# johnmartinsson/differentiable-mel-spectrogram

Measured on AMD Instinct MI355X. Metric: spectrogram frames/sec (fwd+bwd), higher is better.
Workload: dtype f32

## Files before the change

differentiable-mel-spectrogram_amd/build.py:

```python
from __future__ import annotations

import glob
import os
import shutil
import subprocess
import sys

PKG_DIR = os.path.dirname(os.path.abspath(__file__))
CSRC = os.path.join(PKG_DIR, "csrc")
LIB_PATH = os.path.join(PKG_DIR, "libdmel_hip.so")
TORCH_LIB_PATH = os.path.join(PKG_DIR, "libdmel_torch.so")
OBJ_DIR = os.path.join(PKG_DIR, "build")
SPLIT_SOURCES = ["dmel_fwd.hip", "dmel_fwd_len.hip", "dmel_fwd_band.hip", "dmel_fwd_multi_len.hip", "dmel_fwd_band_len.hip", "dmel_fwd_fb_len.hip"]
FWD_PARTS = 4
SOURCES = SPLIT_SOURCES + ["dmel_aux.hip", "dmel_big.hip", "dmel_xgrad.hip", "dmel_xgrad_len.hip", "dmel_xgrad_band.hip", "dmel_xgrad_klen.hip", "dmel_pcen.hip", "dmel_bandnorm.hip", "dmel_specmask.hip", "dmel_deltas.hip", "dmel_statspool.hip", "dmel_attnpool.hip", "dmel_api.cpp", "dmel_tables.cpp", "dmel_comm.cpp"]
PUBLIC_HEADER = os.path.join(os.path.dirname(PKG_DIR), "include", "dmel.h")
HEADERS = sorted(glob.glob(os.path.join(CSRC, "*.h")) + glob.glob(os.path.join(CSRC, "*.inc"))) + [PUBLIC_HEADER]
FLAGS = ["--offload-arch=gfx950", "-O3", "-fPIC", "-std=c++17", "-Wall", "-Wno-unused-function"]


def _hipcc() -> str:
    for cand in (os.environ.get("HIPCC"), shutil.which("hipcc"), "/opt/rocm/bin/hipcc"):
        if cand and os.path.exists(cand):
            return cand
    raise RuntimeError("hipcc not found (set HIPCC or install ROCm)")


def _stale(target: str, deps) -> bool:
    if not os.path.exists(target):
        return True
    t = os.path.getmtime(target)
    return any(os.path.getmtime(d) > t for d in deps)


def _units():
    for src in SOURCES:
        sp = os.path.join(CSRC, src)
        stem = os.path.splitext(src)[0]
        if src in SPLIT_SOURCES:
            for k in range(FWD_PARTS):
                yield sp, os.path.join(OBJ_DIR, f"{stem}_part{k}.o"), ["-DDMEL_FWD_SPLIT", f"-DDMEL_FWD_PART={k}"]
        else:
            yield sp, os.path.join(OBJ_DIR, stem + ".o"), []


def _reap(procs) -> None:
    for pr in procs:
        if pr.poll() is None:
            pr.kill()
    for pr in procs:
        pr.wait()


def build(force: bool = False, verbose: bool = False) -> str:
    os.makedirs(OBJ_DIR, exist_ok=True)
    hipcc = _hipcc()
    objs, running = [], []
    jobs = max(1, min(int(os.environ.get("DMEL_BUILD_JOBS", "0")) or (os.cpu_count() or 2), 8))
    for sp, obj, extra in _units():
        objs.append(obj)
        if force or _stale(obj, [sp] + HEADERS):
            cmd = [hipcc] + FLAGS + extra + ["-x", "hip", "-c", sp, "-o", obj]
            if verbose:
                print(" ".join(cmd), flush=True)
            while len(running) >= jobs:
                if running.pop(0).wait() != 0:
                    _reap(running)
                    raise RuntimeError("hipcc failed")
            running.append(subprocess.Popen(cmd))
    while running:
        if running.pop(0).wait() != 0:
            _reap(running)
            raise RuntimeError("hipcc failed")
    if force or _stale(LIB_PATH, objs):
        cmd = [hipcc, "--offload-arch=gfx950", "-shared", "-fPIC", "-o", LIB_PATH] + objs + ["-ldl"]
        if verbose:
            print(" ".join(cmd), flush=True)
        subprocess.check_call(cmd)
    build_torch(force=force, verbose=verbose)
    return LIB_PATH


def build_torch(force: bool = False, verbose: bool = False) -> str:
    import importlib.util
    spec = importlib.util.find_spec("torch")
    if spec is None or not spec.submodule_search_locations:
        raise RuntimeError("torch is not importable: libdmel_torch.so cannot be built")
    tdir = list(spec.submodule_search_locations)[0]
    src = os.path.join(CSRC, "dmel_torch.cpp")
    if not (force or _stale(TORCH_LIB_PATH, [src, PUBLIC_HEADER, LIB_PATH])):
        return TORCH_LIB_PATH
    cxx = os.environ.get("CXX") or shutil.which("g++") or shutil.which("c++")
    if not cxx:
        raise RuntimeError("no C++ compiler found for libdmel_torch.so")
    inc = os.path.join(tdir, "include")
    cmd = [cxx, "-O2", "-fPIC", "-shared", "-std=c++17", "-D__HIP_PLATFORM_AMD__=1", "-DUSE_ROCM=1", "-D_GLIBCXX_USE_CXX11_ABI=1",
           "-I" + inc, "-I" + os.path.join(inc, "torch", "csrc", "api", "include"), "-I/opt/rocm/include",
           src, "-o", TORCH_LIB_PATH, "-L" + PKG_DIR, "-ldmel_hip", "-L" + os.path.join(tdir, "lib"),
# ... 10 lines not shown
```

differentiable-mel-spectrogram_amd/csrc/dmel_api.cpp:

```cpp
#include "../../include/dmel.h"
#include "dmel_kernels.h"
#include "dmel_lamtrack.h"
#include "dmel_stage.h"
#include "dmel_tables.h"

#include <algorithm>
#include <cmath>
#include <cstdio>
#include <cstdlib>
#include <cstring>
#include <functional>
#include <initializer_list>
#include <map>
#include <mutex>
#include <string>
#include <unordered_set>
#include <vector>

namespace {

thread_local std::string g_err;

dmel_status fail(dmel_status st, const std::string& msg)
{
// ... 432 lines not shown
    bp.split = split ? 1 : 0; bp.wodd = wodd;
    DMEL_HIP(dmel::launch_big(bp, s));
    prof_span(pl, m1, prof_mark(pl, s), 1);
    info->kernel_path = 3; info->frames_per_tile = pair ? 2 : 1; info->grid_fwd = grid;
    info->fb_blocks = 0; info->fb_blocks_dense = 0; info->lds_bytes = dmel::big_uses_global(bt.M) ? 0 : bt.M * 8;
    info->contraction = -1; info->wl_steps = 0;
    return DMEL_OK;
}

dmel_status forward_naive(dmel_plan* pl, NfftTables* tb, const dmel::LamArgs& lam, const FwdCall& c, const Scratch& sc, hipStream_t s,
                          dmel_plan_info* info)
{
    const int N = tb->n_fft;
    dmel::NaiveParams np{};
    np.x = c.x_direct(); np.x_ind = c.x_cell(); np.out = c.out; np.tangent = c.tangent; np.psum = sc.psum; np.win2 = sc.win; np.fb = tb->fb_dense;
    np.B = c.batch; np.L = pl->cfg.n_points; np.T = pl->T; np.hop = pl->cfg.hop_length; np.M = pl->cfg.n_mels;
    np.nchunks = pl->nchunks; np.N = N; np.F = tb->F; np.mode = c.mode;
    np.inv_L = 1.0f / (float)pl->cfg.n_points; np.eps = (float)c.eps; np.flags = c.flags; np.remove_dc = c.remove_dc; np.lam = lam;
    DMEL_HIP(dmel::launch_naive(np, s));
    info->kernel_path = 1; info->frames_per_tile = 1; info->grid_fwd = c.batch * pl->T;
    info->fb_blocks = 0; info->fb_blocks_dense = 0; info->lds_bytes = (2 * N + 2 * tb->F) * 4;
    info->contraction = -1; info->wl_steps = 0;
    return DMEL_OK;
}

dmel_status forward_fused(dmel_plan* pl, NfftTables* tb, const dmel::LamArgs& lam, const FwdCall& c, const Scratch& sc, hipStream_t s,
                          bool kernel_mean, dmel_plan_info* info)
{
    const int N = tb->n_fft;
    const MultiLaunch* ml = c.multi() ? &c.ml : nullptr;
    int mode = c.mode;
    const unsigned flags = c.flags & ~DMEL_FLAG_X_INDIRECT;
    dmel::FwdParams fp{};
    fp.x = c.x_direct(); fp.x_ind = c.x_cell(); fp.out = c.out; fp.tangent = c.tangent; fp.psum = (c.remove_dc && !kernel_mean) ? sc.psum : nullptr; fp.win2 = sc.win;
    fp.tw1 = dmel::mode_pairs(mode) ? tb->tw1p : tb->tw1; fp.tw2 = dmel::mode_pairs(mode) ? tb->tw2p : tb->tw2; fp.ent_b = tb->ent_b; fp.tile_ranges = tb->tile_ranges; fp.ent_b_floats = tb->ent_b_floats; fp.ent_pre = tb->ent_pre;
    for (int i = 0; i < 16; ++i) fp.pre_groups[i] = tb->pre_groups[i];
    fp.B = c.batch; fp.L = pl->cfg.n_points; fp.T = pl->T; fp.hop = pl->cfg.hop_length; fp.M = pl->cfg.n_mels;
    fp.nchunks = pl->nchunks; fp.groups = tb->groups; fp.xch_groups = tb->xch_groups;
    const bool hsplit = (flags & DMEL_FLAG_MFMA_BF16X3) && mode == dmel::kTrain && tb->ent_h != nullptr && (!c.lengths || c.fb_len);
    if (hsplit) mode = dmel::kTrainH;
    static const int wlc_env = std::getenv("DMEL_WLC") ? std::atoi(std::getenv("DMEL_WLC")) : -1;
    const bool wl_compact = tb->wl_total4 * 4 <= 320;
    if (mode == dmel::kTrain && tb->wl_b4 != nullptr && wlc_env != 0 && (wl_compact || wlc_env > 0)) {
        const int wide_fpt = dmel::forward_has_wlc_wide(N) ? dmel::forward_frames_per_tile(N, dmel::kTrainWW) : 0;
        const bool wide = wide_fpt > 0 && wlc_env == 2 && !c.lengths;
        mode = wide ? dmel::kTrainWW : dmel::kTrainW;
        fp.wl_b4 = tb->wl_b4; fp.wl_lane = tb->wl_lane; fp.wl_phases = tb->wl_phases; fp.wl_total4 = tb->wl_total4;
        for (int i = 0; i < dmel::kWlMaxPhases; ++i) { fp.wl_len4[i] = tb->wl_len4[i]; fp.wl_mg[i] = tb->wl_mg[i]; }
        fp.wl_merge = tb->wl_merge;
    }
    const int fpt = dmel::forward_frames_per_tile(N, mode);
    fp.tiles_per_clip = (pl->T + fpt - 1) / fpt;
    fp.inv_L = 1.0f / (float)pl->cfg.n_points; fp.eps = (float)c.eps; fp.flags = flags; fp.lam = lam;
    fp.remove_dc = c.remove_dc; fp.normalize = pl->cfg.normalize_window; fp.win_half = c.win_half;
    fp.spec_out = c.spec_out;
    fp.ent_h = tb->ent_h; fp.fb_nyq = tb->fb_nyq;
    static const int force_tpw = std::getenv("DMEL_TILES_PER_WG") ? std::atoi(std::getenv("DMEL_TILES_PER_WG")) : 0;
    int tpw = dmel::forward_tiles_per_wg(N, mode, c.batch, fp.tiles_per_clip);
    if (force_tpw == 1 || (force_tpw == 2 && dmel::forward_two_tiles(N, mode))) tpw = force_tpw;
    if (hsplit || c.lengths || (ml && ml->edges)) tpw = 1;
    fp.wgs_per_clip = (fp.tiles_per_clip + tpw - 1) / tpw;
    long long grid = (long long)c.batch * fp.wgs_per_clip;
    if (ml) {
        fp.ch_out = ml->ch_out; fp.ch_grid = (int)grid; fp.ch_list = ml->list; fp.ch_roles = ml->roles;
        for (int ch = 0; ch < dmel::kMaxChannels; ++ch) fp.ch_val[ch] = ml->vals[ch];
        grid *= ml->count;
    }
    if (grid > 0x7fffffffLL) return fail(DMEL_ERR_INVALID_ARGUMENT, "too many tiles for one launch");
    if (grid <= dmel::forward_resident_workgroups(N, mode)) fp.flags |= dmel::kFwdEdgeFirst;
    const bool band = ml && ml->edges;
    dmel::FwdLenParams lp{};
    lp.lengths = c.lengths;
    dmel::FwdMultiLenParams mlp{};
    mlp.lengths = c.lengths;
    dmel::FwdBandParams bp{};
    dmel::FwdBandLenParams blp{};
    blp.lengths = c.lengths;
    dmel::FwdFbLenParams flp{};
    flp.lengths = c.lengths;
    const bool fbk = c.fb_len && !ml && (mode == dmel::kTrain || mode == dmel::kTrainH || mode == dmel::kSpec);
    if (c.lengths && c.spec_out && !fbk) return fail(DMEL_ERR_UNSUPPORTED, "per-clip lengths: the spectrogram is saved by the kTrain / kTrainH kernels of a trained bank only");
    for (int ch = 0; band && ch <= dmel::kMaxChannels; ++ch) blp.band_edges[ch] = bp.band_edges[ch] = ml->edges[std::min(ch, ml->channels)];
    auto launch = [&](auto& q) { static_cast<dmel::FwdParams&>(q) = fp; return dmel::launch_forward(N, mode, tpw, q, (int)grid, s); };
    DMEL_HIP(c.lengths ? (band ? launch(blp) : ml ? launch(mlp) : fbk ? launch(flp) : launch(lp)) : band ? launch(bp) : launch(fp));
    info->kernel_path = 0; info->frames_per_tile = fpt; info->grid_fwd = (int)grid;
    info->fb_blocks = tb->n_entries; info->fb_blocks_dense = tb->n_dense;
    info->lds_bytes = dmel::forward_lds_bytes(N, mode);
    const bool spec_only = mode == dmel::kSpec || mode == dmel::kSpecTrain;
    info->contraction = spec_only ? -1 : (dmel::mode_wlc(mode) ? 1 : (mode == dmel::kTrainH ? 2 : 0));
    info->wl_steps = dmel::mode_wlc(mode) ? 4 * fp.wl_total4 : 0;
    return DMEL_OK;
}

dmel_status launch_forward_n(dmel_plan* pl, int N, const dmel::LamArgs& lam, const FwdCall& c, const Scratch& sc, hipStream_t s, bool* sums_done)
{
    if (N < 1) return fail(DMEL_ERR_UNSUPPORTED, "n_fft = " + std::to_string(N));
    const bool pow2 = (N & (N - 1)) == 0;
    const bool big = !pow2 || N > dmel::kMaxNfft;
    if (c.lengths && (big || N < dmel::kMinFastNfft || ((c.spec_out || c.mode == dmel::kSpec) && !c.fb_len) || c.win_half))
        return fail(DMEL_ERR_UNSUPPORTED, "per-clip lengths run the fused kernel only: n_fft 32 ... 16384 (n_fft = " + std::to_string(N) + ")");
    if (c.multi() && (big || N < dmel::kMinFastNfft || c.spec_out))
        return fail(DMEL_ERR_UNSUPPORTED, "the multi-window layer runs n_fft 32 ... 16384 only (n_fft = " + std::to_string(N) + ")");
    if (c.spec_out && (big || N < dmel::kMinFastNfft || c.mode != dmel::kTrain))
        return fail(DMEL_ERR_UNSUPPORTED, "the spectrogram is saved by the fused training kernel only (power-of-two n_fft from 32 to 16384, tangent requested)");
    if (big && (N & 1)) return fail(DMEL_ERR_UNSUPPORTED, "n_fft = " + std::to_string(N) + " is odd");
    NfftTables* tb = nullptr;
    dmel_status st = build_tables(pl, N, &tb);
    if (st != DMEL_OK) return st;
    dmel_plan_info info{};
    info.n_fft = N; info.n_freqs = tb->F; info.n_time = pl->T;
    if (big) {
        if ((st = forward_big(pl, tb, lam, c, sc, s, sums_done, &info)) == DMEL_OK) pl->info = info;
        return st;
    }
    const bool fast = N >= dmel::kMinFastNfft && N <= dmel::kMaxFastNfft;
    const bool kernel_mean = fast && pl->cfg.n_points <= 32768;
    const bool need_sums = c.remove_dc && !kernel_mean && !*sums_done;
    const bool need_window = !fast || !dmel::forward_window_in_lds(N);
    const size_t m0 = prof_mark(pl, s);
    if (need_sums || need_window) {
        if ((st = forward_prep(pl, N, sc.win, lam, c, sc, s, (need_sums ? kPrepSums : 0u) | (need_window ? kPrepWindow : 0u))) != DMEL_OK) return st;
        if (need_sums) *sums_done = true;
    }
    const size_t m1 = prof_mark(pl, s);
    if (need_sums || need_window) prof_span(pl, m0, m1, 0);
    pl->info.n_fft = info.n_fft; pl->info.n_freqs = info.n_freqs; pl->info.n_time = info.n_time;
    st = N < dmel::kMinFastNfft ? forward_naive(pl, tb, lam, c, sc, s, &info) : forward_fused(pl, tb, lam, c, sc, s, kernel_mean, &info);
    if (st != DMEL_OK) return st;
    prof_span(pl, m1, prof_mark(pl, s), 1);
    pl->info = info;
    return DMEL_OK;
}

template <class F> dmel_status issue_group(dmel_plan* pl, int nl, F&& launch)
{
    dmel_plan_info primary_info = pl->info;
    for (int i = 0; i < nl; ++i) {
        const dmel_status st = launch(i);
        if (st != DMEL_OK) return st;
        if (i == 0) primary_info = pl->info;
    }
    pl->info = primary_info;
    return DMEL_OK;
}

dmel_status mailbox_status(const dmel_plan* pl)
{
    const unsigned long long w = dmel::mailbox_peek_error(pl->mailbox);
    if (w == 0) return DMEL_OK;
    return fail(DMEL_ERR_MAILBOX_TIMEOUT, "mailbox all-reduce: rank " + std::to_string((unsigned)(w & 0xffffffffu)) + " never arrived at exchange " +
                std::to_string((unsigned)(w >> 32)) + ": the reduced gradient of that step was NaN on this rank (dmel_mailbox_error clears this)");
}

dmel_status check_device(const dmel_plan* pl)
{
    int dev = -1;
    if (hipGetDevice(&dev) != hipSuccess) { (void)hipGetLastError(); return fail(DMEL_ERR_NO_DEVICE, "no current HIP device"); }
    if (dev != pl->device)
        return fail(DMEL_ERR_INVALID_ARGUMENT, "the plan belongs to device " + std::to_string(pl->device) + " but the current device is " +
                    std::to_string(dev) + " (hipSetDevice / torch.cuda.device before the call)");
    return DMEL_OK;
}

struct StorePtr { const char* name; const void* ptr; };
dmel_status check_store_aligned(const char* fn, std::initializer_list<StorePtr> ptrs)
{
// ... 2179 lines not shown
```

differentiable-mel-spectrogram_amd/csrc/dmel_kernels.h:

```cpp
#pragma once
#include <hip/hip_runtime.h>
#include <stdint.h>
#include <initializer_list>

namespace dmel {

constexpr int kWave = 64;
constexpr int kThreads = 256;
constexpr int kMaxChunks = 64;
constexpr int kMaxFastNfft = 16384;
constexpr int kMaxNfft = 16384;
constexpr int kMinFastNfft = 32;

__device__ __forceinline__ unsigned short bf16_bits(float v) { return __builtin_bit_cast(unsigned short, (__bf16)v); }

enum Mode : int { kTrain = 0, kInfer = 1, kSpec = 2, kSpecTrain = 3,
                  kTrainH = 4,
                  kTrainW = 5,
                  kTrainWW = 6 };
constexpr bool mode_wlc(int mode) { return mode == kTrainW || mode == kTrainWW; }
#ifndef DMEL_WLC_4096
#define DMEL_WLC_4096 0
#endif
#ifndef DMEL_WLC_512
// ... 242 lines not shown
        case 128: f(IC<128>{}); return true;
        case 256: f(IC<256>{}); return true;
        case 512: f(IC<512>{}); return true;
        case 1024: f(IC<1024>{}); return true;
        case 2048: f(IC<2048>{}); return true;
        case 4096: f(IC<4096>{}); return true;
        case 8192: f(IC<8192>{}); return true;
        case 16384: f(IC<16384>{}); return true;
    }
    return false;
}

struct FwdParams {
    const float* x;
    const float* const* x_ind;
    float* out;
    float* tangent;
    const float* psum;
    const float2* win2;
    const float2* tw1;
    const float2* tw2;
    const float* ent_b;
    const int4* tile_ranges;
    int ent_b_floats;
    const float* ent_pre;
    int pre_groups[16];
    int B, L, T, hop, M, nchunks, groups, tiles_per_clip;
    float inv_L, eps;
    LamArgs lam;
    unsigned flags;
    int remove_dc, normalize;
    int win_half;
    int wgs_per_clip;
    unsigned xch_groups;
    const uint4* ent_h;
    const float* fb_nyq;
    float* spec_out;
    const float4* wl_b4;
    const int2* wl_lane;
    int wl_phases, wl_total4;
    int wl_len4[kWlMaxPhases];
    const int* wl_merge;
    int wl_mg[kWlMaxPhases];
    int ch_out, ch_grid;
    unsigned ch_list, ch_roles;
    float ch_val[kMaxChannels];
};

struct FwdLenParams : FwdParams {
    const int* lengths;
};

struct FwdBandParams : FwdParams {
    int band_edges[kMaxChannels + 1];
};

struct FwdMultiLenParams : FwdParams {
    const int* lengths;
};
struct FwdBandLenParams : FwdBandParams {
    const int* lengths;
};
struct FwdFbLenParams : FwdParams {
    const int* lengths;
};

struct PrepParams {
    const float* x; float* psum; float2* win2;
    const float* const* x_ind;
    int B, L, nchunks, chunk, N, normalize;
    LamArgs lam;
    int win_half;
    float center;
    const int* lengths;
};

hipError_t launch_prep(const PrepParams& p, hipStream_t s);
hipError_t launch_forward(int n_fft, int mode, int tiles_per_wg, const FwdParams& p, int grid, hipStream_t s);
hipError_t launch_forward(int n_fft, int mode, int tiles_per_wg, const FwdLenParams& p, int grid, hipStream_t s);
hipError_t launch_forward(int n_fft, int mode, int tiles_per_wg, const FwdBandParams& p, int grid, hipStream_t s);
hipError_t launch_forward(int n_fft, int mode, int tiles_per_wg, const FwdMultiLenParams& p, int grid, hipStream_t s);
hipError_t launch_forward(int n_fft, int mode, int tiles_per_wg, const FwdBandLenParams& p, int grid, hipStream_t s);
hipError_t launch_forward(int n_fft, int mode, int tiles_per_wg, const FwdFbLenParams& p, int grid, hipStream_t s);
int forward_tiles_per_wg(int n_fft, int mode, int batch, int tiles_per_clip);
bool forward_two_tiles(int n_fft, int mode);
int forward_lds_bytes(int n_fft, int mode);
int forward_frames_per_tile(int n_fft, int mode);
int forward_waves(int n_fft);
int forward_nbpre(int n_fft);
bool forward_plan_rc(int n_fft, bool pair, int* R, int* C);
bool forward_has_hsplit(int n_fft);
bool forward_has_wlc(int n_fft);
bool forward_wlc_one_frame(int n_fft);
bool forward_has_wlc_wide(int n_fft);
bool forward_window_in_lds(int n_fft);

__device__ __forceinline__ const float* resolve_x(const float* x, const float* const* x_ind)
{
#if defined(__HIPCC__)
    if (x_ind) { typedef const float* cfp; return *(const __attribute__((address_space(4))) cfp*)x_ind; }
#endif
    return x;
}

struct NaiveParams {
    const float* const* x_ind;
    const float* x; float* out; float* tangent; const float* psum; const float2* win2; const float* fb;
    int B, L, T, hop, M, nchunks, N, F, mode;
    float inv_L, eps; unsigned flags; int remove_dc;
    LamArgs lam;
};
hipError_t launch_naive(const NaiveParams& p, hipStream_t s);


constexpr int kMaxBigFft = 1048576;
struct BigParams {
    const float* const* x_ind;
    const float* x; float* out; float* tangent; const float* psum; const float2* win2;
    const float2* tw;
    const float2* chirp;
    const float2* hbr;
    float2* zws;
    const float* fbT; const int2* band;
    int B, L, T, hop, M, nchunks, N, F, mode, Mfft, logM;
    float inv_L, eps; unsigned flags; int remove_dc;
    LamArgs lam;
    int split;
    const float2* wodd;
};
hipError_t launch_big(const BigParams& p, hipStream_t s);
bool big_can_split(int m_half, int n_mels);
bool big_uses_global(int m_fft);
int big_grid(long long units, int m_fft);

struct XgradParams {
    const float* x; const float* psum; const float2* win2; const float2* tw;
    const float* fb;
    const int2* rowband;
    const float4* rowpk;
    int long_rows;
    const float* grad_out;
    const float* out;
    float* frames;
    float* grad_x;
    double* csum;
    int B, L, T, hop, M, nchunks, N, F, logN, remove_dc;
    int tw_in_lds;
    int spec_mode;
    float inv_L;
    const float2* tw1; const float2* tw2;
    int tiles, span, tile_step;
    int own_prep;
    float win_denom;
    const float* lam_dev;
    int check_nfft;
    int tw2_off;
    int win_n;
    const float2* chirp; const float2* hbr; float2* zws; int Mfft, logM;
};
hipError_t launch_xgrad(const XgradParams& p, hipStream_t s);
hipError_t launch_xgrad_big(const XgradParams& p, int grid, hipStream_t s);
hipError_t launch_xgrad_gather(const XgradParams& p, hipStream_t s);
bool xgrad_wave_shape(int n_fft, int n_mels, int win_n, int* frames_per_tile);
int xgrad_chunks(int L);
hipError_t launch_xgrad_frames(const XgradParams& p, hipStream_t s);

// ... 153 lines not shown
long long specmask_waves_per_image(int n_mels, int T, int elem_bytes);
hipError_t launch_specmask_draw(const SpecMaskDrawParams& p, hipStream_t s);
hipError_t launch_specmask_apply(SpecMaskParams p, int elem_bytes, hipStream_t s);

struct DeltasParams {
    const float* in; float* out;
    const int* lengths;
    long long rows, rows_per_clip;
    int T, n, order, include_static, groups;
    double inv_denom;
    int logw, W, halo, step, chunks;
};
long long deltas_waves(long long rows, int T, int n);
hipError_t launch_deltas(DeltasParams p, bool backward, hipStream_t s);

struct StatsPoolParams {
    const float* s;
    const float* g;
    float* y;
    float* ds;
    const int* lengths;
    double* stats;
    int* argmax;
    long long rows, rows_per_clip;
    int T, which, S;
    double eps;
    int W, logw;
};
hipError_t launch_statspool(StatsPoolParams p, bool backward, hipStream_t s);

struct AttnPoolParams {
    const float* s;
    const float* a;
    const float* g;
    float* y;
    float* ds;
    float* da;
    const int* lengths;
    double* stats;
    double* norm;
    long long rows, rows_per_clip, logit_rows, group;
    int T, which, S;
    double eps;
    int W, logw;
    int chunks, logsplit;
    long long owners;
};
long long attnpool_blocks(long long rows, long long rows_per_clip, long long logit_rows, int T, bool backward);
hipError_t launch_attnpool(AttnPoolParams p, bool backward, hipStream_t s);

constexpr int kMailboxMaxWorld = 16;
struct MailboxArgs {
    unsigned long long* peer_inbox[kMailboxMaxWorld];
    unsigned long long* my_inbox;
    unsigned* step;
    unsigned long long* host_error;
    int rank, world;
    unsigned spin_limit;
    unsigned long long timeout_ticks;
};

hipError_t launch_dot(const void* g, int g_bf16, const float* t, long long count, int accumulate, double* partials,
                      unsigned* counter, int max_partials, float* result, hipStream_t s, const MailboxArgs* mb = nullptr,
                      const AdamParams* fused = nullptr);
int dot_multi_blocks_per_channel(long long per_channel, int channels);
hipError_t launch_dot_multi(const void* g, int g_bf16, const float* t, int batch, int channels, long long per_row, int blocks_per_channel,
                            int accumulate, double* partials, unsigned* counter, float* result, hipStream_t s);
struct DotBandParams {
    const void* g; const float* t; double* partials; unsigned* counter; float* result;
    int g_bf16, batch, channels, M, T, accumulate;
    int edges[kMaxChannels + 1];
    int blocks[kMaxChannels];
};
void dot_band_deal(const int* edges, int channels, int batch, int T, int* blocks);
hipError_t launch_dot_band(const DotBandParams& p, hipStream_t s);
hipError_t launch_mailbox_allreduce(float* buf, const MailboxArgs& mb, hipStream_t s);

hipError_t forward_prepare_attributes();
hipError_t forward_len_prepare_attributes();
hipError_t forward_band_prepare_attributes();
hipError_t forward_multi_len_prepare_attributes();
hipError_t forward_band_len_prepare_attributes();
hipError_t forward_fb_len_prepare_attributes();
hipError_t xgrad_prepare_attributes();
hipError_t xgrad_len_prepare_attributes();
hipError_t xgrad_band_prepare_attributes();
hipError_t xgrad_klen_prepare_attributes();
hipError_t big_prepare_attributes();
inline hipError_t prepare_attributes()
{
    for (auto unit : {forward_prepare_attributes, forward_len_prepare_attributes, forward_band_prepare_attributes, forward_multi_len_prepare_attributes,
                      forward_band_len_prepare_attributes, forward_fb_len_prepare_attributes, xgrad_prepare_attributes,
                      xgrad_len_prepare_attributes, xgrad_band_prepare_attributes, xgrad_klen_prepare_attributes, big_prepare_attributes})
        if (const hipError_t e = unit(); e != hipSuccess) return e;
    return hipSuccess;
}

}
```

Measured before the change: 225.1 million.

## Add specialized N=1024 kTrainW forward kernel with fused window, FFT, and MFMA mel contraction

Adds a dedicated forward kernel for n_fft=1024 in the kTrainW mode, with tiles_per_wg=1 and no per-clip lengths. It is hard-specialized to the 32x32 FFT plan and keeps the window table and first-stage twiddles in LDS. The mel contraction is done with MFMA instructions fed by a buffer-load prefetch ring, and outputs are staged in LDS before coalesced float4 stores. The intent is to drop the generic template's runtime branching and improve load/compute overlap for this common configuration. The cost is a large block of duplicated code, paths that only some parameter combinations can take, and an XCD-aware workgroup remap.

```diff
diff --git a/differentiable-mel-spectrogram_amd/build.py b/differentiable-mel-spectrogram_amd/build.py
--- a/differentiable-mel-spectrogram_amd/build.py
+++ b/differentiable-mel-spectrogram_amd/build.py
@@ -13,7 +13,7 @@
 OBJ_DIR = os.path.join(PKG_DIR, "build")
 SPLIT_SOURCES = ["dmel_fwd.hip", "dmel_fwd_len.hip", "dmel_fwd_band.hip", "dmel_fwd_multi_len.hip", "dmel_fwd_band_len.hip", "dmel_fwd_fb_len.hip"]
 FWD_PARTS = 4
-SOURCES = SPLIT_SOURCES + ["dmel_aux.hip", "dmel_big.hip", "dmel_xgrad.hip", "dmel_xgrad_len.hip", "dmel_xgrad_band.hip", "dmel_xgrad_klen.hip", "dmel_pcen.hip", "dmel_bandnorm.hip", "dmel_specmask.hip", "dmel_deltas.hip", "dmel_statspool.hip", "dmel_attnpool.hip", "dmel_api.cpp", "dmel_tables.cpp", "dmel_comm.cpp"]
+SOURCES = SPLIT_SOURCES + ["dmel_w1024.hip", "dmel_aux.hip", "dmel_big.hip", "dmel_xgrad.hip", "dmel_xgrad_len.hip", "dmel_xgrad_band.hip", "dmel_xgrad_klen.hip", "dmel_pcen.hip", "dmel_bandnorm.hip", "dmel_specmask.hip", "dmel_deltas.hip", "dmel_statspool.hip", "dmel_attnpool.hip", "dmel_api.cpp", "dmel_tables.cpp", "dmel_comm.cpp"]
 PUBLIC_HEADER = os.path.join(os.path.dirname(PKG_DIR), "include", "dmel.h")
 HEADERS = sorted(glob.glob(os.path.join(CSRC, "*.h")) + glob.glob(os.path.join(CSRC, "*.inc"))) + [PUBLIC_HEADER]
 FLAGS = ["--offload-arch=gfx950", "-O3", "-fPIC", "-std=c++17", "-Wall", "-Wno-unused-function"]
diff --git a/differentiable-mel-spectrogram_amd/csrc/dmel_api.cpp b/differentiable-mel-spectrogram_amd/csrc/dmel_api.cpp
--- a/differentiable-mel-spectrogram_amd/csrc/dmel_api.cpp
+++ b/differentiable-mel-spectrogram_amd/csrc/dmel_api.cpp
@@ -538,6 +538,8 @@
     if (c.lengths && c.spec_out && !fbk) return fail(DMEL_ERR_UNSUPPORTED, "per-clip lengths: the spectrogram is saved by the kTrain / kTrainH kernels of a trained bank only");
     for (int ch = 0; band && ch <= dmel::kMaxChannels; ++ch) blp.band_edges[ch] = bp.band_edges[ch] = ml->edges[std::min(ch, ml->channels)];
     auto launch = [&](auto& q) { static_cast<dmel::FwdParams&>(q) = fp; return dmel::launch_forward(N, mode, tpw, q, (int)grid, s); };
+    if (dmel::forward_w1024_takes(N, mode, tpw, fp, !c.lengths && !ml)) DMEL_HIP(dmel::launch_forward_w1024(fp, (int)grid, s));
+    else
     DMEL_HIP(c.lengths ? (band ? launch(blp) : ml ? launch(mlp) : fbk ? launch(flp) : launch(lp)) : band ? launch(bp) : launch(fp));
     info->kernel_path = 0; info->frames_per_tile = fpt; info->grid_fwd = (int)grid;
     info->fb_blocks = tb->n_entries; info->fb_blocks_dense = tb->n_dense;
diff --git a/differentiable-mel-spectrogram_amd/csrc/dmel_kernels.h b/differentiable-mel-spectrogram_amd/csrc/dmel_kernels.h
--- a/differentiable-mel-spectrogram_amd/csrc/dmel_kernels.h
+++ b/differentiable-mel-spectrogram_amd/csrc/dmel_kernels.h
@@ -348,6 +348,8 @@
 hipError_t launch_forward(int n_fft, int mode, int tiles_per_wg, const FwdMultiLenParams& p, int grid, hipStream_t s);
 hipError_t launch_forward(int n_fft, int mode, int tiles_per_wg, const FwdBandLenParams& p, int grid, hipStream_t s);
 hipError_t launch_forward(int n_fft, int mode, int tiles_per_wg, const FwdFbLenParams& p, int grid, hipStream_t s);
+bool forward_w1024_takes(int n_fft, int mode, int tiles_per_wg, const FwdParams& p, bool scalar_launch);
+hipError_t launch_forward_w1024(const FwdParams& p, int grid, hipStream_t s);
 int forward_tiles_per_wg(int n_fft, int mode, int batch, int tiles_per_clip);
 bool forward_two_tiles(int n_fft, int mode);
 int forward_lds_bytes(int n_fft, int mode);
@@ -667,6 +669,7 @@
 hipError_t forward_multi_len_prepare_attributes();
 hipError_t forward_band_len_prepare_attributes();
 hipError_t forward_fb_len_prepare_attributes();
+hipError_t forward_w1024_prepare_attributes();
 hipError_t xgrad_prepare_attributes();
 hipError_t xgrad_len_prepare_attributes();
 hipError_t xgrad_band_prepare_attributes();
@@ -675,7 +678,7 @@
 inline hipError_t prepare_attributes()
 {
     for (auto unit : {forward_prepare_attributes, forward_len_prepare_attributes, forward_band_prepare_attributes, forward_multi_len_prepare_attributes,
-                      forward_band_len_prepare_attributes, forward_fb_len_prepare_attributes, xgrad_prepare_attributes,
+                      forward_band_len_prepare_attributes, forward_fb_len_prepare_attributes, forward_w1024_prepare_attributes, xgrad_prepare_attributes,
                       xgrad_len_prepare_attributes, xgrad_band_prepare_attributes, xgrad_klen_prepare_attributes, big_prepare_attributes})
         if (const hipError_t e = unit(); e != hipSuccess) return e;
     return hipSuccess;
diff --git a/differentiable-mel-spectrogram_amd/csrc/dmel_w1024.hip b/differentiable-mel-spectrogram_amd/csrc/dmel_w1024.hip
--- /dev/null
+++ b/differentiable-mel-spectrogram_amd/csrc/dmel_w1024.hip
@@ -0,0 +1,444 @@
+#include <cstdint>
+#include <cstdlib>
+
+#include "dmel_kernels.h"
+#include "dmel_wavefft.h"
+
+#ifndef DMEL_WL_DEPTH
+#define DMEL_WL_DEPTH 6
+#endif
+#ifndef DMEL_TW1_CHUNK
+#define DMEL_TW1_CHUNK 4
+#endif
+
+namespace dmel {
+
+#include "dmel_fwd_log.h"
+
+namespace {
+constexpr int kN = 1024;
+constexpr FftGeom kG = geom_mode<kN, kTrainW>();
+static_assert(kG.R == 32 && kG.C == 1 && kG.G == 32 && kG.FPW == 2 && kG.PASSES == 1 && kG.WPF == 1 && kG.WAVES == 8 && kG.SLOTS == 16,
+              "dmel_w1024_kernel is written for the 32 x 32 plan: two frames per wave, 16 per workgroup");
+static_assert(kG.PAIRING == kPairBperm && kG.SPLIT != 0 && kG.WIN_LDS != 0 && kG.WIN_SYM != 0 && kG.TW1_OFF != 0,
+              "... with the compact layout, the half window table and the first-stage twiddles in LDS");
+constexpr bool kW1024Default = true;
+}
+
+__global__ void __launch_bounds__(kG.THREADS, kG.MINW) dmel_w1024_kernel(FwdParams p)
+{
+    constexpr FftGeom g = kG;
+    constexpr int N = kN, R = g.R, G = g.G, FPW = g.FPW, SLOTS = g.SLOTS, WAVES = g.WAVES, THREADS = g.THREADS;
+    constexpr int LB = ilog2(R);
+    constexpr int EXS = g.EX_STRIDE, SS = g.SLOT_STRIDE_F2;
+    constexpr int FPT = SLOTS;
+    constexpr int F = N / 2 + 1;
+    static_assert(THREADS == N / 2, "one window entry per thread");
+
+    extern __shared__ __attribute__((aligned(16))) unsigned char smem_raw[];
+    v2f* lds = reinterpret_cast<v2f*>(smem_raw);
+    float2* wtab = reinterpret_cast<float2*>(smem_raw + g.AUX_OFF);
+    float* red = reinterpret_cast<float*>(smem_raw + g.RED_OFF);
+
+    const int tid = threadIdx.x;
+    const int lane = tid & 63;
+    const int wave = __builtin_amdgcn_readfirstlane(tid >> 6);
+    int wg = blockIdx.x;
+    {
+        const int nwg = gridDim.x, q = nwg >> 3, rr = nwg & 7, xcd = wg & 7;
+        wg = (xcd < rr ? xcd * (q + 1) : rr * (q + 1) + (xcd - rr) * q) + (wg >> 3);
+    }
+    const int b = wg / p.wgs_per_clip;
+    const int tile0 = wg % p.wgs_per_clip;
+    const float* xbase = p.x;
+    if (p.x_ind) { typedef const float* cfp; xbase = *(const __attribute__((address_space(4))) cfp*)p.x_ind; }
+    const __amdgpu_buffer_rsrc_t rx = make_rsrc(xbase + (size_t)b * p.L, (unsigned)p.L * 4u);
+
+    constexpr int WL_DEPTH = DMEL_WL_DEPTH;
+    floatx4 wl_ring[WL_DEPTH];
+    const __amdgpu_buffer_rsrc_t rbw = make_rsrc((const void*)p.wl_b4, (unsigned)p.wl_total4 * 1024u);
+    auto wl_bload = [&](floatx4& dst, int grp, int n4, int boff4) {
+        const int gi = boff4 + grp < n4 ? boff4 + grp : n4;
+        dst = __builtin_bit_cast(floatx4, __builtin_amdgcn_raw_buffer_load_b128(rbw, lane * 16, __builtin_amdgcn_readfirstlane(gi) * 1024, 0));
+    };
+    auto wl_last = [&](int n4, int boff4) -> int {
+        int l = boff4 + n4; l = l < p.wl_total4 ? l : p.wl_total4; l -= 1;
+        return l > 0 ? l : 0;
+    };
+    auto wl_ring_init = [&](int n4, int boff4) {
+        n4 = wl_last(n4, boff4);
+        static_for<0, WL_DEPTH>([&](auto dd) { constexpr int d = decltype(dd)::value; asm volatile("" : "=v"(wl_ring[d])); wl_bload(wl_ring[d], d, n4, boff4); });
+    };
+
+    const int j = lane / G;
+    const int lg = lane % G;
+    const int qp = lg;
+    auto sync_frame = [&]() {
+        __builtin_amdgcn_fence(__ATOMIC_RELEASE, "wavefront");
+        __builtin_amdgcn_wave_barrier();
+        __builtin_amdgcn_fence(__ATOMIC_ACQUIRE, "wavefront");
+    };
+
+    const float lam_raw = lam_load(p.lam);
+    const int t0 = tile0 * FPT;
+    const int slot = wave * FPW + j;
+    const int tA = t0 + slot;
+    const int f0 = tA * p.hop - N / 2;
+    float xa[R];
+    const bool inside = __all((f0 >= 0) && (f0 + N <= p.L));
+    {
+        const int sA = f0 + lg;
+        if (inside) {
+            static_for<0, R>([&](auto aa) {
+                constexpr int a = decltype(aa)::value;
+                xa[a] = buf_f32(rx, (sA + G * a) * 4);
+            });
+        } else {
+            static_for<0, R>([&](auto aa) {
+                constexpr int a = decltype(aa)::value;
+                xa[a] = buf_f32(rx, clampi(sA + G * a, p.L - 1) * 4);
+            });
+        }
+    }
+
+    float mean = 0.f;
+    if ((p.flags & kFwdEdgeFirst) && !inside) __builtin_amdgcn_s_setprio(2);
+    const LamState ls0 = lam_prologue(p.lam, N, blockIdx.x == 0 && tid == 0, lam_raw);
+    const LamState ls = lam_clip_scale(ls0, p.L);
+    if (ls.action != kLamRun) {
+        if (ls.action == kLamPoison) {
+            const float qn = __builtin_nanf("");
+            for (int idx = tid; idx < p.M * FPT; idx += THREADS) {
+                const int rr = idx / FPT, t = t0 + idx % FPT;
+                if (t >= p.T) continue;
+                const size_t o = ((size_t)b * p.M + rr) * p.T + t;
+                p.out[o] = qn;
+                p.tangent[o] = qn;
+            }
+        }
+        return;
+    }
+    if (wave == 0) { const float h = 0.5f * lam_tangent_scale(ls); if (lane == 0) red[kRedTan] = h; }
+    {
+        constexpr int n16 = (R - 1) * G / 2;
+        for (int i = tid; i < n16; i += THREADS)
+            reinterpret_cast<float4*>(smem_raw + g.TW1_OFF)[i] = reinterpret_cast<const float4*>(p.tw1 + G)[i];
+    }
+    {
+        constexpr int first = 2 * F, count = SS * 2 - first;
+        static_assert(count > 0, "slot stride covers PD[0 .. N/2] and its padding");
+        constexpr int CP = 1 << (ilog2(count - 1 > 0 ? count - 1 : 1) + 1);
+        static_assert(count <= CP, "slot padding fits the zeroing loop");
+        for (int i = tid; i < SLOTS * CP; i += THREADS) {
+            const int sl_z = i / CP, jz = i % CP;
+            if (jz < count) reinterpret_cast<float*>(smem_raw + sl_z * (SS * 8))[first + jz] = 0.f;
+        }
+    }
+    {
+        const float denom = ls.denom;
+        const int n = tid;
+        const float d = (float)n - (float)N / 2.0f;
+        const float t = d / denom;
+        const float w = expf(-0.5f * (t * t));
+        const float dw = w * (d * d) * ls.s2;
+        wtab[n] = make_float2(w, dw);
+        if (tid == 0) wtab[N / 2] = make_float2(1.f, 0.f);
+    }
+    auto mean_of = [&](float wsum) -> float {
+        if (lane == 0) red[wave] = wsum;
+        __syncthreads();
+        float t[WAVES];
+        static_for<0, WAVES>([&](auto qq) { t[decltype(qq)::value] = red[decltype(qq)::value]; });
+        static_for<0, ilog2(WAVES)>([&](auto ll) {
+            constexpr int st = 1 << decltype(ll)::value;
+            static_for<0, WAVES / (2 * st)>([&](auto ii) { constexpr int i = decltype(ii)::value * 2 * st; t[i] += t[i + st]; });
+        });
+        return mean_quotient(t[0], p.L, p.inv_L);
+    };
+    if (p.tiles_per_clip == 1) {
+        float ps = 0.f;
+        static_for<R / 2, R>([&](auto aa) {
+            constexpr int a = decltype(aa)::value;
+            const int n = lg + G * a;
+            const bool seg = n < N / 2 + p.hop;
+            const int ia = slot * p.hop - N / 2 + n;
+            ps += (seg && slot < p.T && ia < p.L) ? xa[a] : 0.f;
+        });
+        mean = mean_of(wave_sum(ps));
+    } else {
+        const float* xc = xbase + (size_t)b * p.L;
+        float a0 = 0.f, a1 = 0.f, a2 = 0.f, a3 = 0.f;
+        int i = 0;
+        constexpr int KB = 8;
+        if ((reinterpret_cast<uintptr_t>(xc) & 15) == 0) {
+            const float4* x4 = reinterpret_cast<const float4*>(xc);
+            const int n4 = p.L / 4;
+            for (int base = 0; base < n4; base += THREADS * KB) {
+                float4 v[KB];
+                static_for<0, KB>([&](auto jj) {
+                    constexpr int jv = decltype(jj)::value;
+                    const int q = base + tid + THREADS * jv;
+                    v[jv] = x4[q < n4 ? q : n4 - 1];
+                });
+                static_for<0, KB>([&](auto jj) {
+                    constexpr int jv = decltype(jj)::value;
+                    const float okf = (base + tid + THREADS * jv < n4) ? 1.f : 0.f;
+                    a0 = fmaf(v[jv].x, okf, a0); a1 = fmaf(v[jv].y, okf, a1); a2 = fmaf(v[jv].z, okf, a2); a3 = fmaf(v[jv].w, okf, a3);
+                });
+            }
+            i = n4 * 4;
+        }
+        for (int base = i; base < p.L; base += THREADS * KB) {
+            float v[KB];
+            static_for<0, KB>([&](auto jj) { v[decltype(jj)::value] = buf_f32(rx, (base + tid + THREADS * decltype(jj)::value) * 4); });
+            static_for<0, KB>([&](auto jj) { a0 += v[decltype(jj)::value]; });
+        }
+        mean = mean_of(wave_sum((a0 + a1) + (a2 + a3)));
+    }
+
+    {
+        v2f* sl = lds + slot * SS;
+        v2f z[R];
+        int wbyte = g.AUX_OFF + lg * 8;
+        int wbyte_m = g.AUX_OFF + (G - lg) * 8;
+        asm volatile("" : "+v"(wbyte), "+v"(wbyte_m));
+        auto wload = [&](auto aa_) -> v2f {
+            constexpr int a = decltype(aa_)::value;
+            float2 wd2;
+            if constexpr (a >= R / 2) wd2 = *reinterpret_cast<const float2*>(smem_raw + wbyte_m + G * 8 * (R - 1 - a));
+            else wd2 = *reinterpret_cast<const float2*>(smem_raw + wbyte + G * 8 * a);
+            return v2f{wd2.x, wd2.y};
+        };
+        float va_last;
+        v2f wd_last;
+        if (inside) {
+            const float mean_i = mean;
+            static_for<0, R>([&](auto aa) {
+                constexpr int a = decltype(aa)::value;
+                const v2f wd = wload(aa);
+                const float va = xa[a] - mean_i;
+                if constexpr (a == R - 1) { va_last = va; wd_last = wd; }
+                else z[a] = splat(va) * wd;
+            });
+        } else {
+            static_for<0, R>([&](auto aa) {
+                constexpr int a = decltype(aa)::value;
+                const int n = lg + G * a;
+                const v2f wd = wload(aa);
+                const int ia = f0 + n;
+                const float va = ((ia >= 0) && (ia < p.L)) ? xa[a] - mean : 0.f;
+                if constexpr (a == R - 1) { va_last = va; wd_last = wd; }
+                else z[a] = splat(va) * wd;
+            });
+        }
+        z[R - 1] = splat(va_last) * wd_last;
+        fft_reg_dit<R>(z);
+        v2f u[R];
+        int tw1b = g.TW1_OFF + lg * 8;
+        asm volatile("" : "+v"(tw1b));
+        {
+            float* slf = reinterpret_cast<float*>(sl);
+            constexpr int TW1C = DMEL_TW1_CHUNK;
+            float2 tw1r[R];
+            auto tw1_fetch = [&](auto cc) {
+                constexpr int c0 = decltype(cc)::value;
+                static_for<(c0 == 0 ? 1 : c0), (c0 + TW1C < R ? c0 + TW1C : R)>([&](auto q1) {
+                    constexpr int q = decltype(q1)::value;
+                    tw1r[q] = *reinterpret_cast<const float2*>(smem_raw + tw1b + (q - 1) * (G * 8));
+                });
+            };
+            tw1_fetch(IC<0>{});
+            __builtin_amdgcn_sched_barrier(0);
+            static_for<0, R>([&](auto qq) {
+                constexpr int q = decltype(qq)::value;
+                v2f v;
+                if constexpr (q % TW1C == 0 && q + TW1C < R) {
+                    __builtin_amdgcn_sched_barrier(0);
+                    tw1_fetch(IC<q + TW1C>{});
+                    __builtin_amdgcn_sched_barrier(0);
+                }
+                v = z[bitrev(q, LB)];
+                if constexpr (q != 0) v = cmul(v, tw1r[q]);
+                z[bitrev(q, LB)] = v;
+                slf[q * EXS + lg] = v.x;
+            });
+            sync_frame();
+            float ure[R];
+            static_for<0, R>([&](auto bb) {
+                constexpr int bi = decltype(bb)::value;
+                ure[bi] = slf[qp * EXS + bi];
+            });
+            sync_frame();
+            static_for<0, R>([&](auto qq) {
+                constexpr int q = decltype(qq)::value;
+                slf[q * EXS + lg] = z[bitrev(q, LB)].y;
+            });
+            sync_frame();
+            static_for<0, R>([&](auto bb) {
+                constexpr int bi = decltype(bb)::value;
+                u[bi] = v2f{ure[bi], slf[qp * EXS + bi]};
+            });
+            sync_frame();
+        }
+        fft_reg_dit<R>(u);
+        v2f zr[R];
+        static_for<0, R>([&](auto pp1) {
+            constexpr int p1 = decltype(pp1)::value;
+            zr[p1] = u[bitrev(p1, LB)];
+        });
+        {
+            const bool q0 = (qp == 0);
+            const int fl0 = j * G;
+            const int pull = (fl0 + ((R - qp) & (R - 1))) * 4;
+            const int slot_b = slot * (SS * 8);
+            const int base_a = slot_b + qp * 8;
+            static_for<0, R / 2 + 1>([&](auto pp1) {
+                constexpr int p1 = decltype(pp1)::value;
+                constexpr int s_a = (p1 == R / 2) ? R / 2 : (R - 1 - p1);
+                constexpr int s_b = (p1 == R / 2) ? R / 2 : ((R - p1) % R);
+                const float send_x = (s_a == s_b) ? zr[s_a].x : (q0 ? zr[s_b].x : zr[s_a].x);
+                const float send_y = (s_a == s_b) ? zr[s_a].y : (q0 ? zr[s_b].y : zr[s_a].y);
+                const int got_x = __builtin_amdgcn_ds_bpermute(pull, __builtin_bit_cast(int, send_x));
+                const int got_y = __builtin_amdgcn_ds_bpermute(pull, __builtin_bit_cast(int, send_y));
+                const v2f zn = v2f{__builtin_bit_cast(float, got_x), __builtin_bit_cast(float, got_y)};
+                const v2f zk = zr[p1];
+                float sx = zk.x + zn.x, sy = zk.y - zn.y, dx = zk.x - zn.x, dy = zk.y + zn.y;
+                const v2f pdv = v2f{fmaf(sx, sx, sy * sy), fmaf(sx, dy, -(sy * dx))};
+                if constexpr (p1 < R / 2) *reinterpret_cast<v2f*>(smem_raw + base_a + R * 8 * p1) = pdv;
+                else { if (q0) *reinterpret_cast<v2f*>(smem_raw + base_a + R * 8 * (R / 2)) = pdv; }
+            });
+            __builtin_amdgcn_sched_barrier(0);
+        }
+    }
+    sync_frame();
+    const float htan = red[kRedTan];
+
+    const bool do_log = (p.flags & 1u) != 0;
+    const int row = lane & 3;
+    const int fr = row & 1, typ = row >> 1;
+    const int a_lane = (wave * FPW + fr) * (SS * 8) + typ * 4;
+    int off4 = 0;
+    float* const out_clip = p.out + (size_t)b * p.M * p.T;
+    float* const tan_clip = p.tangent + (size_t)b * p.M * p.T;
+    constexpr int NST = 2;
+    float sv[NST][2 * FPW];
+    int sm[NST];
+    static_for<0, NST>([&](auto pp) { sm[decltype(pp)::value] = -1; });
+    int2 li_pref = p.wl_lane[lane];
+    for (int ph = 0; ph < p.wl_phases; ++ph) {
+        const int n4 = p.wl_len4[ph];
+        const int2 li = li_pref;
+        if (ph + 1 < p.wl_phases) li_pref = p.wl_lane[(ph + 1) * 64 + lane];
+        if (ph == 0) wl_ring_init(n4, off4);
+        off4 += n4;
+        int aaddr = a_lane + li.x;
+        floatx4 acc0 = {0.f, 0.f, 0.f, 0.f}, acc1 = {0.f, 0.f, 0.f, 0.f};
+        float a_cur[4];
+        static_for<0, 4>([&](auto uu) { constexpr int u = decltype(uu)::value; a_cur[u] = *reinterpret_cast<const float*>(smem_raw + aaddr + 8 * u); });
+        auto group = [&](auto dd) {
+            constexpr int d = decltype(dd)::value;
+            float a_nxt[4];
+            static_for<0, 4>([&](auto uu) { constexpr int u = decltype(uu)::value; a_nxt[u] = *reinterpret_cast<const float*>(smem_raw + aaddr + 32 * (d + 1) + 8 * u); });
+            const floatx4 bq = wl_ring[d];
+            acc0 = __builtin_amdgcn_mfma_f32_4x4x1f32(a_cur[0], bq[0], acc0, 0, 0, 0);
+            acc1 = __builtin_amdgcn_mfma_f32_4x4x1f32(a_cur[1], bq[1], acc1, 0, 0, 0);
+            acc0 = __builtin_amdgcn_mfma_f32_4x4x1f32(a_cur[2], bq[2], acc0, 0, 0, 0);
+            acc1 = __builtin_amdgcn_mfma_f32_4x4x1f32(a_cur[3], bq[3], acc1, 0, 0, 0);
+            static_for<0, 4>([&](auto uu) { constexpr int u = decltype(uu)::value; a_cur[u] = a_nxt[u]; });
+        };
+        int s4 = 0;
+        const int ring_n4 = wl_last(n4, off4 - n4);
+        for (; s4 + WL_DEPTH <= n4; s4 += WL_DEPTH) {
+            static_for<0, WL_DEPTH>([&](auto dd) {
+                constexpr int d = decltype(dd)::value;
+                group(dd);
+                wl_bload(wl_ring[d], s4 + d + WL_DEPTH, ring_n4, off4 - n4);
+                __builtin_amdgcn_sched_group_barrier(0x100, 2, 0);
+                __builtin_amdgcn_sched_group_barrier(0x008, 4, 0);
+                __builtin_amdgcn_sched_group_barrier(0x020, 1, 0);
+            });
+            aaddr += WL_DEPTH * 32;
+        }
+        static_for<0, WL_DEPTH - 1>([&](auto dd) { if (s4 + decltype(dd)::value < n4) group(dd); });
+        if (ph + 1 < p.wl_phases) wl_ring_init(p.wl_len4[ph + 1], off4);
+        const floatx4 tot = acc0 + acc1;
+        const int m = li.y;
+        if (m < 0) continue;
+        float ov[FPW], tv[FPW];
+        static_for<0, FPW>([&](auto ff) {
+            constexpr int f = decltype(ff)::value;
+            const float mel = 0.25f * tot[f];
+            const float dmel = htan * tot[2 + f];
+            const float me = mel + p.eps;
+            ov[f] = do_log ? fast_log(me, p.eps) : mel;
+            tv[f] = do_log ? dmel * __builtin_amdgcn_rcpf(me) : dmel;
+        });
+        static_for<0, NST>([&](auto pp) {
+            if (decltype(pp)::value == ph) {
+                sm[decltype(pp)::value] = m;
+                static_for<0, FPW>([&](auto ff) { constexpr int f = decltype(ff)::value; sv[decltype(pp)::value][f] = ov[f]; sv[decltype(pp)::value][FPW + f] = tv[f]; });
+            }
+        });
+    }
+    {
+        float* const stg = reinterpret_cast<float*>(smem_raw + wave * FPW * (SS * 8));
+        static_for<0, NST>([&](auto pp) {
+            constexpr int q = decltype(pp)::value;
+            if (sm[q] >= 0) {
+                static_for<0, 2>([&](auto tt2) {
+                    constexpr int pl = decltype(tt2)::value;
+                    float* d = stg + ((pl * p.M + sm[q]) * FPW);
+                    *reinterpret_cast<float2*>(d) = make_float2(sv[q][pl * FPW], sv[q][pl * FPW + 1]);
+                });
+            }
+        });
+        __syncthreads();
+        constexpr int QPR = SLOTS / 4;
+        const int srows = p.M;
+        const int total = 2 * srows * QPR;
+        const unsigned img_bytes = (unsigned)p.M * (unsigned)p.T * 4u;
+        const __amdgpu_buffer_rsrc_t r_out = make_rsrc(out_clip, img_bytes);
+        const __amdgpu_buffer_rsrc_t r_tan = make_rsrc(tan_clip, img_bytes);
+        for (int idx = tid; idx < total; idx += THREADS) {
+            const int rw = idx / QPR, c = idx % QPR;
+            const int pl = rw >= srows ? 1 : 0, mm = rw - pl * srows;
+            const float2 lo = *reinterpret_cast<const float2*>(smem_raw + (2 * c) * FPW * (SS * 8) + ((pl * p.M + mm) * FPW) * 4);
+            const float2 hi = *reinterpret_cast<const float2*>(smem_raw + (2 * c + 1) * FPW * (SS * 8) + ((pl * p.M + mm) * FPW) * 4);
+            const float4 v = make_float4(lo.x, lo.y, hi.x, hi.y);
+            const int t = t0 + 4 * c;
+            if (t + 3 < p.T) {
+                const unsigned eo = (unsigned)mm * (unsigned)p.T + t0 + 4 * c;
+                if (pl == 0) buf_store_wt_f4(r_out, eo * 4u, v);
+                else buf_store_wt_f4(r_tan, eo * 4u, v);
+            }
+        }
+    }
+}
+
+bool forward_w1024_takes(int n_fft, int mode, int tpw, const FwdParams& p, bool scalar_launch)
+{
+    static const bool on = [] { const char* e = std::getenv("DMEL_W1024"); return e != nullptr ? std::atoi(e) != 0 : kW1024Default; }();
+    if (!on || !scalar_launch || n_fft != kN || mode != kTrainW || tpw != 1 || p.ch_out != 0) return false;
+    if (p.tangent == nullptr || p.out == nullptr || p.spec_out != nullptr || p.psum != nullptr) return false;
+    if ((p.flags & ~(1u | kFwdEdgeFirst)) != 0) return false;
+    if (!p.remove_dc || p.normalize || p.win_half) return false;
+    if (p.hop < 1 || p.hop > kN / 2 || p.L < 1 || p.T < 4 || (p.T & 3) != 0 || p.M < 1) return false;
+    if (p.wl_b4 == nullptr || p.wl_lane == nullptr || p.wl_phases < 1 || p.wl_phases > 2 || p.wl_total4 < 1 || p.M > kG.SLOT_STRIDE_F2) return false;
+    if ((unsigned long long)p.M * (unsigned long long)p.T * 4ull > 0xffffffffull) return false;
+    if (((reinterpret_cast<uintptr_t>(p.out) | reinterpret_cast<uintptr_t>(p.tangent)) & 15) != 0) return false;
+    if (p.x_ind == nullptr && (reinterpret_cast<uintptr_t>(p.x) & 15) != 0) return false;
+    return true;
+}
+
+hipError_t launch_forward_w1024(const FwdParams& p, int grid, hipStream_t s)
+{
+    hipLaunchKernelGGL(dmel_w1024_kernel, dim3(grid), dim3(kG.THREADS), kG.LDS_BYTES, s, p);
+    return hipGetLastError();
+}
+
+hipError_t forward_w1024_prepare_attributes()
+{
+    return hipFuncSetAttribute(reinterpret_cast<const void*>(dmel_w1024_kernel), hipFuncAttributeMaxDynamicSharedMemorySize, kG.LDS_BYTES);
+}
+
+}
```

Result: no change. 226.8 million (median of 6 runs) (+0.8%).
